# prstrive/SuRF

Hardware: AMD Instinct MI355X
Metric: rays/sec (576x800, 5-view, 128 samp/ray render, whole job) (higher is better)
Workload: dtype f32 (operands split exactly into 3 bf16 pieces, fp32 accumulate)

## Files before the change

include/surf_hip.h:

```cpp
#ifndef SURF_HIP_H
#define SURF_HIP_H

#include <stdint.h>

#ifdef __cplusplus
extern "C" {
#endif

#define SURF_MAX_VIEWS 8
#define SURF_MAX_STAGES 4
#define SURF_MAX_SAMPLES 256

#define SURF_E_ARG (-1)
#define SURF_E_LIMIT (-2)

#define SURF_ABI_VERSION 41
int surf_abi_version(void);

int surf_pack_texel4(const float* src, int n, int C, int H, int W, float* dst, void* stream);

int surf_ray_setup(const float* rays_o, const float* rays_d, const float* near, const float* far, int n_rays,
                   const float* mvol, int Dm, const float* lin_depth, int n_depth, const float* lin_samples,
                   const int* h_n_samples, const float* h_sample_ranges, int n_stage, const float* jitter,
                   float sample_dist, const int32_t* const* h_tables, const int* h_dims, int n_vol,
// ... 84 lines not shown
int surf_sdf_smooth_backward(const float* pts, const float* sbar, int64_t n, const float* const* h_vols,
                             const int32_t* const* h_tables, const int* h_dims, int n_vol, float* const* h_dvols,
                             const float* packed, float* in, float* ab, void* stream);

int surf_blend_raw_floats(void);
int surf_blend_packed_floats(void);
int surf_blend_pack_weights(const float* h_raw, float* h_packed);
int surf_blend(const float* pts, const uint8_t* mask, const int32_t* idx, int64_t n, const float* const* h_feats, const int* h_hw,
               int n_level, const float* imgs, int nv, const float* h_intrs, const float* h_w2c,
               const float* h_c2w, const float* blend_w, float* color, uint8_t* n_valid, void* stream);

#define SURF_BLEND_BF16X3 1
#define SURF_BLEND_F16X2 2
#define SURF_BLEND_F32 3
int64_t surf_blend_split_packed_bytes(int precision);
int surf_blend_pack_weights_split(const float* h_raw, unsigned char* h_packed, int precision);
int64_t surf_blend_split_scratch_bytes(int64_t n_points, int nv);
int surf_blend_split(const float* pts, const uint8_t* mask, const int32_t* idx, int64_t n, const float* const* h_feats,
                     const int* h_hw, int n_level, const float* imgs, int nv, const float* h_intrs, const float* h_w2c,
                     const float* h_c2w, const void* blend_w, int precision, float* color, uint8_t* n_valid, void* scratch,
                     void* stream);
int surf_blend_split_dn(const float* pts, const int32_t* idx, int64_t n_capacity, const int32_t* d_n, const float* const* h_feats,
                        const int* h_hw, int n_level, const float* imgs, int nv, const float* h_intrs, const float* h_w2c,
                        const float* h_c2w, const void* blend_w, int precision, float* color, uint8_t* n_valid, void* scratch,
                        void* stream);

int surf_composite(const float* sdf, const float* grad, const float* color, const uint8_t* n_valid,
                   const float* mid_z, const float* dists, const float* pts, const uint8_t* vmask,
                   const float* rays_d, int n_rays, int S, float inv_s, float cos_anneal_ratio,
                   const float* h_rot_ref, float* out_color, float* out_depth, float* out_sdf_depth,
                   float* out_normal, float* out_normal_val, uint8_t* out_valid, uint8_t* out_mid_inside,
                   float* out_weights, float* out_inside, float* out_eik, float* out_z_sdf0, void* stream);
int surf_composite_backward(const float* sdf, const float* grad, const float* color, const float* mid_z, const float* dists,
                            const float* pts, const uint8_t* vmask, const float* rays_d, int n_rays, int S, float inv_s,
                            float cos_anneal_ratio, const float* h_rot_ref, const float* g_color, const float* g_depth,
                            float eik_scale, float* d_sdf, float* d_grad, float* d_color, float* d_inv_s, void* stream);
int surf_composite_backward_s(const float* sdf, const float* grad, const float* color, const float* mid_z, const float* dists,
                              const float* pts, const uint8_t* vmask, const float* rays_d, int n_rays, int S, float inv_s,
                              float cos_anneal_ratio, const float* h_rot_ref, const float* g_color, const float* g_depth,
                              float eik_scale, const float* eik_upstream, float* d_sdf, float* d_grad, float* d_color,
                              float* d_inv_s, void* stream);



int surf_upsample_filter(const int32_t* parents, int64_t n_parents, int D, const float* depths, int nv, int H, int W,
                         const float* h_intrs, const float* h_w2c, float depth_range, uint8_t* flags, void* stream);

int surf_costvol(const int32_t* parents, const int32_t* idx, int64_t n, int D, const float* const* h_feats,
                 const int* h_hw, int stage, int nv, const float* h_intrs, const float* h_w2c, const float* h_agg,
                 int32_t* coords, float* feat, uint8_t* keep, void* stream);

int64_t surf_compact_workspace_ints(int64_t n);
int surf_compact(const uint8_t* flags, int64_t n, int32_t* workspace, int32_t* idx_out, int32_t* total, void* stream);

int surf_gather_rows(const void* src, const int32_t* idx, int64_t n, int row_words, int idx_shift, int dst_stride_words,
                     int dst_offset_words, void* dst, void* stream);
int surf_compose_index(const int32_t* a, const int32_t* b, int64_t n, int32_t* out, void* stream);

int surf_densify(const int32_t* coords, const float* rows, int row_stride, int64_t n, int D, const float* prev,
                 float* dense, int32_t* table, void* stream);

int surf_matching_depth(const float* mvol, int D, int nv, const float* h_kinv, const float* h_c2w, const float* h_rinv,
                        const float* h_near_fars, int H, int W, int h, int w, const float* lin_x, const float* lin_y,
                        const float* lin_n, int n, const float* pre_depths, float ratio_cur, float ratio_prev,
                        const float* jitter, float* depth_lr, float* depth_full, float* stats, void* stream);


int surf_spconv(const float* in, int cin, const int32_t* in_table, int D_in, const int32_t* out_coords, int64_t n_out,
                int mode, const float* weight, int cout, const float* bn_scale, const float* bn_shift, const float* skip,
                float* out, void* stream);
int surf_spconv_rows16(const uint16_t* in16, int cin, const int32_t* in_table, int D_in, const int32_t* out_coords, int64_t n_out,
                       int mode, const float* weight, int cout, float* out, void* stream);
int surf_rows_to_bf16(const float* x, int64_t n_floats, uint16_t* out16, void* stream);
int surf_bn_relu_apply16(const float* x, int64_t n, int channels, const float* scale, const float* shift, const float* skip,
                         float* out, uint16_t* out16, void* stream);
int surf_bn_relu_backward16(const float* x, const float* dy, int64_t n, int channels, const float* scale, const float* shift,
                            const float* mean, const float* invstd, int train, void* workspace, float* dgamma, float* dbeta,
                            float* dx, uint16_t* dx16, void* stream);
int64_t surf_spconv_packed_bytes(int cin, int cout);
int surf_spconv_pack_weights(const float* weight, int cin, int cout, void* packed, void* stream);
int surf_spconv_mfma(const float* in, int cin, const int32_t* in_table, int D_in, const int32_t* out_coords, int64_t n_out,
                     int mode, const void* packed, int cout, const float* bn_scale, const float* bn_shift,
                     const float* skip, float* out, int bf16_operands, void* stream);

int64_t surf_bn_workspace_bytes(int channels);
int surf_bn_train_affine(const float* x, int64_t n, int channels, const float* gamma, const float* beta, float eps,
                         float momentum, float* running_mean, float* running_var, float* scale, float* shift, float* batch_stats,
                         void* workspace, void* stream);
int surf_bn_relu_apply(const float* x, int64_t n, int channels, const float* scale, const float* shift, const float* skip,
                       float* out, void* stream);
int surf_bn_relu_backward(const float* x, const float* dy, int64_t n, int channels, const float* scale, const float* shift,
                          const float* mean, const float* invstd, int train, void* workspace, float* dgamma, float* dbeta,
                          float* dx, void* stream);
int64_t surf_inorm_backward_workspace_bytes(int N, int channels);
int surf_inorm_relu_backward(const float* x, const float* dy, int N, int64_t hw, int channels, const float* stats, void* workspace,
                             float* dx, void* stream);

int surf_matching_depth_backward(const float* mvol, int D, int nv, const float* h_kinv, const float* h_c2w, const float* h_rinv,
                                 const float* h_near_fars, int H, int W, int h, int w, const float* lin_x, const float* lin_y,
                                 const float* lin_n, int n, const float* pre_depths, float ratio_cur, float ratio_prev,
                                 const float* jitter, const float* g_full, int view0, int view1, float* g_lr, float* dmvol,
                                 const float* stats, void* stream);
int surf_densify_backward(const int32_t* coords, int64_t n, int D, const int32_t* table, const float* g_dense, int row_stride,
                          float* g_rows, float* g_prev, void* stream);
int surf_scatter_rows_add(const float* g_dst, const int32_t* idx, int64_t n, int row_words, int idx_shift, int dst_stride_words,
                          int dst_offset_words, float* g_src, void* stream);
// ... 162 lines not shown
```

surf_amd/csrc/volume.hip:

```cpp
#include <stdlib.h>

#include "common.h"

namespace {

struct ViewSet {
  int nv;
  float w2c[SURF_MAX_VIEWS][12];
  float K[SURF_MAX_VIEWS][12];
};

__constant__ int kChildOff[8][3] = {{0, 0, 0}, {1, 0, 0}, {0, 1, 0}, {0, 0, 1}, {1, 1, 0}, {1, 0, 1}, {0, 1, 1}, {1, 1, 1}};

__device__ __forceinline__ bool project_voxel(const ViewSet& vs, int v, float wx, float wy, float wz, float half_w,
                                              float half_h, float& nx, float& ny, float& qz) {
  const float* M = vs.w2c[v];
  float X = M[0] * wx + M[1] * wy + M[2] * wz + M[3];
  float Y = M[4] * wx + M[5] * wy + M[6] * wz + M[7];
  float Z = M[8] * wx + M[9] * wy + M[10] * wz + M[11];
  const float* K = vs.K[v];
  float qx = K[0] * X + K[1] * Y + K[2] * Z + K[3];
  float qy = K[4] * X + K[5] * Y + K[6] * Z + K[7];
  qz = K[8] * X + K[9] * Y + K[10] * Z + K[11];
  float x = qx / qz, y = qy / qz;
// ... 178 lines not shown
  __syncthreads();
  if (threadIdx.x == 0) block_counts[blockIdx.x] = s_part[0] + s_part[1] + s_part[2] + s_part[3];
}

__global__ __launch_bounds__(1024) void compact_scan_kernel(int32_t* __restrict__ block_counts, int nb,
                                                            int32_t* __restrict__ total) {
  __shared__ int s_buf[1024];
  __shared__ int s_carry;
  if (threadIdx.x == 0) s_carry = 0;
  __syncthreads();
  for (int c0 = 0; c0 < nb; c0 += 1024) {
    const int i = c0 + threadIdx.x;
    const int v = i < nb ? block_counts[i] : 0;
    s_buf[threadIdx.x] = v;
    __syncthreads();
    for (int o = 1; o < 1024; o <<= 1) {
      int t = threadIdx.x >= o ? s_buf[threadIdx.x - o] : 0;
      __syncthreads();
      s_buf[threadIdx.x] += t;
      __syncthreads();
    }
    const int incl = s_buf[threadIdx.x];
    const int carry = s_carry;
    if (i < nb) block_counts[i] = carry + incl - v;
    __syncthreads();
    if (threadIdx.x == 1023) s_carry = carry + incl;
    __syncthreads();
  }
  if (threadIdx.x == 0) *total = s_carry;
}

__global__ __launch_bounds__(CP_THREADS) void compact_scatter_kernel(const uint8_t* __restrict__ flags, int64_t n,
                                                                     const int32_t* __restrict__ block_offsets,
                                                                     int32_t* __restrict__ idx_out, bool aligned) {
  __shared__ int s_part[CP_THREADS / 64];
  const int lane = threadIdx.x & 63, wave = threadIdx.x >> 6;
  const int64_t base = (int64_t)blockIdx.x * CP_BLOCK + (int64_t)threadIdx.x * CP_ITEMS;
  const unsigned bits = cp_mask16(flags, base, n, aligned);
  const int c = __popc(bits);
  int incl = c;
#pragma unroll
  for (int o = 1; o < 64; o <<= 1) {
    int t = __shfl_up(incl, o);
    if (lane >= o) incl += t;
  }
  if (lane == 63) s_part[wave] = incl;
  __syncthreads();
  int wave_off = 0;
  for (int w = 0; w < wave; ++w) wave_off += s_part[w];
  int pos = block_offsets[blockIdx.x] + wave_off + incl - c;
#pragma unroll
  for (int k = 0; k < CP_ITEMS; ++k)
    if (bits & (1u << k)) idx_out[pos++] = (int32_t)(base + k);
}

__global__ __launch_bounds__(256) void gather_rows_kernel(const uint32_t* __restrict__ src, const int32_t* __restrict__ idx,
                                                          int64_t n, int w, int shift, int dst_stride, int dst_off,
                                                          uint32_t* __restrict__ dst) {
  const int64_t t = (int64_t)blockIdx.x * blockDim.x + threadIdx.x;
  if (t >= n * w) return;
  const int64_t i = t / w;
  const int c = (int)(t % w);
  dst[i * dst_stride + dst_off + c] = src[(int64_t)(idx[i] >> shift) * w + c];
}

__global__ __launch_bounds__(256) void compose_index_kernel(const int32_t* __restrict__ a, const int32_t* __restrict__ b,
                                                            int64_t n, int32_t* __restrict__ out) {
  const int64_t i = (int64_t)blockIdx.x * blockDim.x + threadIdx.x;
  if (i < n) out[i] = a[b[i]];
}

__device__ __forceinline__ void up2_src(int i, int Dp, int& i0, int& i1, float& l1) {
  float src = ((float)i + 0.5f) * 0.5f - 0.5f;
  if (src < 0.f) src = 0.f;
  i0 = (int)floorf(src);
  i1 = min(i0 + 1, Dp - 1);
  l1 = src - (float)i0;
}

template <int VEC, int NV>
__global__ __launch_bounds__(256) void dense_init_kernel(const float* __restrict__ prev, int D, float* __restrict__ dense,
                                                         int32_t* __restrict__ table) {
  const int64_t total = (int64_t)D * D * D;
  const int64_t t0 = (int64_t)blockIdx.x * (256 * NV) + threadIdx.x;
  const unsigned zc = (unsigned)D / VEC;
#pragma unroll
  for (int k = 0; k < NV; ++k) {
    const int64_t t = t0 + 256 * k, i0 = t * VEC;
    if (i0 >= total) return;
    const unsigned tu = (unsigned)t;
    const int zb = (int)(tu % zc) * VEC, y = (int)((tu / zc) % (unsigned)D), x = (int)(tu / (zc * (unsigned)D));
    float out[VEC];
    if (VEC == 4 && prev) {
      const int Dp = D / 2;
      int x0, x1, y0, y1;
      float lx, ly;
      up2_src(x, Dp, x0, x1, lx);
      up2_src(y, Dp, y0, y1, ly);
      const float hx = 1.0f - lx, hy = 1.0f - ly;
      const int c0 = zb / 2 - 1;
      float P[4][4];
#pragma unroll
      for (int t = 0; t < 4; ++t) {
        const int zc = min(max(c0 + t, 0), Dp - 1);
        P[0][t] = prev[((int64_t)x0 * Dp + y0) * Dp + zc];
        P[1][t] = prev[((int64_t)x0 * Dp + y1) * Dp + zc];
// ... 561 lines not shown
extern "C" int surf_upsample_filter(const int32_t* parents, int64_t n_parents, int D, const float* depths, int nv, int H,
                                    int W, const float* h_intrs, const float* h_w2c, float depth_range, uint8_t* flags,
                                    void* stream) {
  if (!parents || !depths || !h_intrs || !h_w2c || !flags || n_parents <= 0 || D < 2 || H < 2 || W < 2) return SURF_E_ARG;
  if (nv < 1 || nv > SURF_MAX_VIEWS) return SURF_E_LIMIT;
  FilterArgs a;
  a.parents = parents; a.n_par = n_parents; a.D = D; a.voxel_size = (float)(2.0 / (double)(D - 1));
  a.depths = depths; a.H = H; a.W = W; a.depth_range = depth_range; a.flags = flags;
  fill_views(a.vs, nv, h_intrs, h_w2c);
  hipLaunchKernelGGL(upsample_filter_kernel, grid1d(n_parents * 8, 256), dim3(256), 0, (hipStream_t)stream, a);
  return surf_check_launch();
}

extern "C" int surf_costvol(const int32_t* parents, const int32_t* idx, int64_t n, int D, const float* const* h_feats,
                            const int* h_hw, int stage, int nv, const float* h_intrs, const float* h_w2c,
                            const float* h_agg , int32_t* coords, float* feat,
                            uint8_t* keep, void* stream) {
  if (!h_feats || !h_hw || !h_intrs || !h_w2c || !h_agg || !coords || !feat || !keep || n <= 0 || D < 2) return SURF_E_ARG;
  if ((idx != nullptr) != (parents != nullptr)) return SURF_E_ARG;
  if (!idx && n != (int64_t)D * D * D) return SURF_E_ARG;
  if (nv < 1 || nv > SURF_MAX_VIEWS || stage < 0 || stage > 3) return SURF_E_LIMIT;
  CostVolArgs a;
  a.parents = parents; a.idx = idx; a.n = n; a.D = D; a.voxel_size = (float)(2.0 / (double)(D - 1)); a.stage = stage;
  for (int l = 0; l < 4; ++l) {
    if (!h_feats[l]) return SURF_E_ARG;
    a.feats[l] = h_feats[l];
    a.hw[2 * l] = h_hw[2 * l];
    a.hw[2 * l + 1] = h_hw[2 * l + 1];
  }
  fill_views(a.vs, nv, h_intrs, h_w2c);
  for (int k = 0; k < 32; ++k) a.w1[k] = h_agg[k];
  for (int k = 0; k < 8; ++k) { a.b1[k] = h_agg[32 + k]; a.w2[k] = h_agg[40 + k]; }
  a.b2 = h_agg[48];
  a.coords = coords; a.feat = feat; a.keep = keep;
  hipLaunchKernelGGL(costvol_kernel, grid1d(n, 256), dim3(256), 0, (hipStream_t)stream, a);
  return surf_check_launch();
}

extern "C" int64_t surf_compact_workspace_ints(int64_t n) { return (n + CP_BLOCK - 1) / CP_BLOCK + 1; }

extern "C" int surf_compact(const uint8_t* flags, int64_t n, int32_t* workspace, int32_t* idx_out, int32_t* total,
                            void* stream) {
  if (!flags || !workspace || !idx_out || !total || n <= 0) return SURF_E_ARG;
  if (n > 0x7fffffffLL) return SURF_E_LIMIT;
  const int nb = (int)((n + CP_BLOCK - 1) / CP_BLOCK);
  hipStream_t st = (hipStream_t)stream;
  const bool aligned = ((uintptr_t)flags & 15u) == 0;
  hipLaunchKernelGGL(compact_count_kernel, dim3(nb), dim3(CP_THREADS), 0, st, flags, n, workspace, aligned);
  hipLaunchKernelGGL(compact_scan_kernel, dim3(1), dim3(1024), 0, st, workspace, nb, total);
  hipLaunchKernelGGL(compact_scatter_kernel, dim3(nb), dim3(CP_THREADS), 0, st, flags, n, workspace, idx_out, aligned);
  return surf_check_launch();
}

extern "C" int surf_gather_rows(const void* src, const int32_t* idx, int64_t n, int row_words, int idx_shift,
                                int dst_stride_words, int dst_offset_words, void* dst, void* stream) {
  if (!src || !idx || !dst || n <= 0 || row_words <= 0 || idx_shift < 0 || dst_stride_words < row_words) return SURF_E_ARG;
  hipLaunchKernelGGL(gather_rows_kernel, grid1d(n * row_words, 256), dim3(256), 0, (hipStream_t)stream,
                     (const uint32_t*)src, idx, n, row_words, idx_shift, dst_stride_words, dst_offset_words, (uint32_t*)dst);
  return surf_check_launch();
}

extern "C" int surf_compose_index(const int32_t* a, const int32_t* b, int64_t n, int32_t* out, void* stream) {
  if (!a || !b || !out || n <= 0) return SURF_E_ARG;
  hipLaunchKernelGGL(compose_index_kernel, grid1d(n, 256), dim3(256), 0, (hipStream_t)stream, a, b, n, out);
  return surf_check_launch();
}

extern "C" int surf_densify(const int32_t* coords, const float* rows, int row_stride, int64_t n, int D, const float* prev,
                            float* dense, int32_t* table, void* stream) {
  if (!coords || !rows || !dense || !table || n <= 0 || D < 2 || row_stride < 1) return SURF_E_ARG;
  if (prev && (D & 1)) return SURF_E_ARG;
  hipStream_t st = (hipStream_t)stream;
  if (D % 4 == 0)
    hipLaunchKernelGGL((dense_init_kernel<4, 4>), grid1d((int64_t)D * D * D / 4, 256 * 4), dim3(256), 0, st, prev, D, dense, table);
  else
    hipLaunchKernelGGL((dense_init_kernel<1, 4>), grid1d((int64_t)D * D * D, 256 * 4), dim3(256), 0, st, prev, D, dense, table);
  hipLaunchKernelGGL(dense_scatter_kernel, grid1d(n, 256), dim3(256), 0, st, coords, rows, row_stride, n, D, dense, table);
  return surf_check_launch();
}

extern "C" int surf_densify_backward(const int32_t* coords, int64_t n, int D, const int32_t* table, const float* g_dense,
                                     int row_stride, float* g_rows, float* g_prev, void* stream) {
  if (!coords || !table || !g_dense || !g_rows || n <= 0 || D < 2 || row_stride < 1) return SURF_E_ARG;
  if (g_prev && (D & 1)) return SURF_E_ARG;
  hipStream_t st = (hipStream_t)stream;
  hipLaunchKernelGGL(dense_rows_bwd_kernel, grid1d(n, 256), dim3(256), 0, st, coords, g_dense, n, D, row_stride, g_rows);
  if (g_prev)
  {
    const int64_t total = (int64_t)D * D * D;
    const int Dp = D / 2;
    const int64_t tiles = (int64_t)((Dp + DG_TX - 1) / DG_TX) * ((Dp + DG_TY - 1) / DG_TY) * ((Dp + DG_TZ - 1) / DG_TZ);
#ifndef SURF_DENSE_BWD_SCATTER
    if (tiles <= 0x7fffffffLL && Dp >= 2)
      hipLaunchKernelGGL(dense_init_bwd_gather_kernel, dim3((unsigned)tiles), dim3(256), 0, st, g_dense, table, D, g_prev);
    else
#endif
    if (D % 4 == 0)
      hipLaunchKernelGGL((dense_init_bwd_kernel<4, 8>), grid1d(total / 4, 256 * 8), dim3(256), 0, st, g_dense, table, D, g_prev);
    else
      hipLaunchKernelGGL((dense_init_bwd_kernel<1, 8>), grid1d(total, 256 * 8), dim3(256), 0, st, g_dense, table, D, g_prev);
  }
  return surf_check_launch();
}

extern "C" int surf_scatter_rows_add(const float* g_dst, const int32_t* idx, int64_t n, int row_words, int idx_shift,
                                     int dst_stride_words, int dst_offset_words, float* g_src, void* stream) {
// ... 88 lines not shown
```

surf_amd/implicit_surface.py:

```python
import math

import numpy as np
import torch
import torch.nn as nn

from . import ops
from .grads import accumulate


class _WNLinear(nn.Module):

    def __init__(self, weight, bias):
        super().__init__()
        self.weight_g = nn.Parameter(torch.linalg.norm(weight, dim=1, keepdim=True).clone())
        self.weight_v = nn.Parameter(weight.clone())
        self.bias = nn.Parameter(bias.clone())


class SDFNetworkSparse(nn.Module):

    def __init__(self, d_in=3, d_out=129, d_hidden=128, n_layers=6, skip_in=(3,), multires=4, bias=0.5, scale=1.0,
                 geometric_init=True, weight_norm=True, inside_outside=False, feat_channels=28, feat_multires=0):
        super().__init__()
        if not (d_in == 3 and d_hidden == 128 and n_layers == 6 and tuple(skip_in) == (3,) and multires == 4
                and feat_channels == 28 and feat_multires == 0 and float(scale) == 1.0 and weight_norm):
            raise NotImplementedError("the HIP SDF kernel implements the architecture shipped in confs/*.conf "
                                      "(d_hidden 128, n_layers 6, skip_in [3], multires 4, feat_channels 28, scale 1)")
        self.scale = scale
        in0 = 3 + 3 * 2 * multires
        dims = [in0] + [d_hidden + feat_channels] * n_layers + [d_out]
        self.num_layers = len(dims)
        for l in range(self.num_layers - 1):
            out_dim = dims[l + 1] - dims[0] if (l + 1) in skip_in else dims[l + 1]
            if l < self.num_layers - 2:
                out_dim -= feat_channels
            lin = nn.Linear(dims[l], out_dim)
            if geometric_init:
                with torch.no_grad():
                    if l == self.num_layers - 2:
                        sgn = -1.0 if inside_outside else 1.0
                        nn.init.normal_(lin.weight, mean=sgn * math.sqrt(math.pi) / math.sqrt(dims[l]), std=0.0001)
                        nn.init.constant_(lin.bias, -sgn * bias)
                        lin.weight[:, -feat_channels:] = 0.0
                        lin.bias[-feat_channels:] = 0.0
                    elif l == 0:
                        nn.init.constant_(lin.bias, 0.0)
                        lin.weight[:, 3:] = 0.0
                        nn.init.normal_(lin.weight[:, :3], 0.0, math.sqrt(2) / math.sqrt(out_dim))
                    elif l in skip_in:
                        nn.init.constant_(lin.bias, 0.0)
                        nn.init.normal_(lin.weight, 0.0, math.sqrt(2) / math.sqrt(out_dim))
                        lin.weight[:, -(dims[0] - 3 + feat_channels):] = 0.0
                    else:
# ... 47 lines not shown
        self.mvol = mv.contiguous().float()
        self.sv = ops.SparseVolumes([v.detach().float() for v in volumes], list(sparse_idxes))
        self.feats_t4 = [ops.pack_texel4(f.detach().float().contiguous()) for f in features]
        self.imgs_t4 = ops.pack_texel4(imgs.detach().float().contiguous())
        self.cams = ops.Cameras(intrs, c2ws)
        self.device = dev
        self.match_feats_t4 = None
        self._warp_maps = {}

    def occupied_any(self, pts):
        return ops.occupied_any(pts.float().contiguous(), self.sv)

    def warp_maps(self, use_match=False):
        key = bool(use_match and self.match_feats_t4 is not None)
        if key and getattr(self, "match_ready", None) is not None:
            ops.side.wait_for(self.match_ready)
            self.match_ready = None
        if key not in self._warp_maps:
            f = self.match_feats_t4 if key else self.feats_t4
            H, W = f[0].shape[1:3]
            self._warp_maps[key] = [f[0], ops.upsample_bilinear_t4(f[1], H, W), ops.upsample_bilinear_t4(f[2], H, W)]
        return self._warp_maps[key]

    @classmethod
    def from_device_layouts(cls, mvol, volumes, tables, feats_t4, imgs_t4, cams):
        self = cls.__new__(cls)
        self.mvol = mvol
        self.sv = ops.SparseVolumes(list(volumes), list(tables))
        self.feats_t4 = list(feats_t4)
        self.imgs_t4 = imgs_t4
        self.cams = cams
        self.device = mvol.device
        self.match_feats_t4 = None
        self._warp_maps = {}
        return self


class _LatticeScene:

    def __init__(self, volumes, sparse_idxes):
        self.sv = ops.SparseVolumes([v.detach().float() for v in volumes], list(sparse_idxes))
        self.device = self.sv.vols[0].device


def _occupied_list(rec, key):
    lst = rec.get(key + "_idx")
    if lst is None:
        lst = rec[key + "_idx"] = rec[key].nonzero().squeeze(1)
    return lst


MESH_EXTRACTIONS = ("dense", "band")
MESH_BAND_MARGIN = 2.0


class ImplicitSurface(nn.Module):

    def __init__(self, confs):
        super().__init__()
        self.n_samples = [int(n) for n in confs.get_list("render.n_samples")]
        self.sample_ranges = [float(r) for r in confs.get_list("render.sample_ranges")]
        self.n_depth = confs.get_int("render.n_depth")
        self.perturb = confs.get_float("render.perturb")
        self.val_chunk = confs.get_int("render.val_chunk", 1 << 19)
        self.sdf_network = SDFNetworkSparse(**dict(confs["sdf_network"]))
        self.color_network = BlendingNetwork(**dict(confs["color_network"]))
        self.deviation_network = SingleVarianceNetwork(**dict(confs["variance_network"]))
        self.sdf_precision = confs.get_string("render.sdf_precision", "bf16x3")
        if self.sdf_precision not in ops.SDF_PRECISIONS:
            raise ValueError(f"render.sdf_precision must be one of {ops.SDF_PRECISIONS}, got {self.sdf_precision!r}")
        self.blend_precision = confs.get_string("render.blend_precision", ops.BLEND_DEFAULT)
        if self.blend_precision not in ops.BLEND_PRECISIONS:
            raise ValueError(f"render.blend_precision must be one of {ops.BLEND_PRECISIONS}, got {self.blend_precision!r}")
        self.mesh_extraction = confs.get_string("render.mesh_extraction", "dense")
        if self.mesh_extraction not in MESH_EXTRACTIONS:
            raise ValueError(f"render.mesh_extraction must be one of {MESH_EXTRACTIONS}, got {self.mesh_extraction!r}")
        self.mesh_band_margin = confs.get_float("render.mesh_band_margin", MESH_BAND_MARGIN)
        if not self.mesh_band_margin >= 0.0:
            raise ValueError(f"render.mesh_band_margin must be >= 0, got {self.mesh_band_margin!r}")
        self.mesh_vertex_attributes = bool(confs.get_bool("render.vertex_attributes", False))
        self._packed = None
        self.kernel_events = None
        self.active_samples_log = None
        self.last_active_samples = None
        self.register_load_state_dict_post_hook(lambda module, incompatible: module.invalidate_packed())

    def invalidate_packed(self):
        self._packed = None
        if getattr(self.sdf_network, "_surf_flat", None) is not None:
            object.__setattr__(self.sdf_network, "_surf_flat", None)

    def train(self, mode=True):
        self.invalidate_packed()
        return super().train(mode)

    def packed_weights(self, device):
        ver = tuple((p._version, p.data_ptr()) for p in self.parameters()) + (str(device), self.sdf_precision, self.blend_precision)
        if self._packed is None or self._packed[0] != ver:
            from . import packing
            on_device = next(self.parameters()).is_cuda and packing.supported(self.sdf_precision, self.blend_precision)
            if on_device:
                with torch.no_grad():
                    sdf_w = packing.sdf_pack_split_device(self.sdf_network, self.sdf_precision)
                    blend_w = packing.blend_pack_split_device(self.color_network, self.blend_precision)
            else:
                sd = {k: v for k, v in self.state_dict().items()}
                sdf_w = (ops.sdf_pack_weights(sd, device, "sdf_network.") if self.sdf_precision == "f32" else
                         ops.sdf_pack_weights_split(sd, device, "sdf_network.", self.sdf_precision))
                blend_w = ops.blend_pack_weights(sd, device, "color_network.", self.blend_precision)
            self._packed = (ver, sdf_w, blend_w)
        return self._packed[1], self._packed[2]

    def smooth_weights(self, device):
        self.packed_weights(device)
        if len(self._packed) == 3:
            if next(self.parameters()).is_cuda:
                from . import packing
                with torch.no_grad():
                    sm = packing.sdf_pack_smooth_device(self.sdf_network)
            else:
                sm = ops.sdf_smooth_pack_weights({k: v for k, v in self.state_dict().items()}, device, "sdf_network.")
            self._packed = self._packed + (sm,)
        return self._packed[3]

    def scene(self, matching_volume, volumes, sparse_idxes, mask_volumes, features, imgs, intrs, c2ws):
        return SceneVolumes(matching_volume, volumes, sparse_idxes, features, imgs, intrs, c2ws)

    def render_scene(self, rays_o, rays_d, near, far, scene, cos_anneal_ratio=1.0, per_sample=True, jitter=None,
                     patch_warp=False, step=None):
        dev = rays_o.device
        self._random_pts = None
        if jitter is None and self.perturb > 0:
            jitter = self.draw_jitter(rays_o.shape[0])
        if jitter is not None:
            jitter = jitter.to(dev, torch.float32).contiguous()
        sdf_w, blend_w = self.packed_weights(dev)
        rays_o = rays_o.float().contiguous()
        rays_d = rays_d.float().contiguous()
        ev = self.kernel_events

        def timed(name, fn):
            if ev is None:
                return fn()
            a, b = torch.cuda.Event(enable_timing=True), torch.cuda.Event(enable_timing=True)
            a.record()
            r = fn()
            b.record()
            ev.append((name, a, b))
            return r

        st = timed("ray_setup", lambda: ops.ray_setup(rays_o, rays_d, near.float(), far.float(), scene.mvol, scene.sv,
                                                      self.n_samples, self.sample_ranges, self.n_depth, jitter=jitter,
                                                      want_z=patch_warp))
        n_act = None
        if patch_warp or self.sdf_precision == "f32" or self.blend_precision == "f32":
            act = timed("compact", lambda: ops.compact(st["vmask"]))
            if patch_warp and act.shape[0] == 0:
                act = torch.arange(min(10, st["vmask"].numel()), dtype=torch.int32, device=dev)
        else:
            act, n_act = timed("compact", lambda: ops.compact_counted(st["vmask"]))
        side_fwd = None
        if patch_warp:
            def smooth_branch():
                smooth, _ = ops.sdf_smooth(st["pts"], scene.sv, self.smooth_weights(dev), active_idx=act)
                inside = ((torch.linalg.norm(st["pts"], ord=2, dim=-1) < 1.0) & st["vmask"].bool()).float()
                err = (torch.linalg.norm(smooth, ord=2, dim=-1) * inside).sum() / (inside.sum() + 1e-5)
                return smooth, inside, err

            def sparse_branch():
                pr = self._random_pts if self._random_pts is not None else torch.rand([1024, 3]) * 2 - 1
                pr = pr.to(dev, torch.float32).contiguous()
                occ = scene.occupied_any(pr)
                sdf_r, _ = ops.sdf_mlp(pr, scene.sv, sdf_w, mask=occ.to(torch.uint8), want_grad=False)
                return pr, occ, torch.where(occ, sdf_r, torch.zeros_like(sdf_r))

            if ops.side.active("fwd") and dev.type == "cuda" and ev is None:
                self.smooth_weights(dev)
                side_fwd = (ops.side.run(smooth_branch, lane=1), ops.side.run(sparse_branch, lane=0))
        sdf, grad = timed("sdf_mlp", lambda: ops.sdf_mlp(st["pts"], scene.sv, sdf_w, mask=st["vmask"], active_idx=act,
                                                         active_count=n_act))
        col, nvalid = timed("blend", lambda: ops.blend(st["pts"], scene.feats_t4, scene.imgs_t4, scene.cams, blend_w,
                                                       mask=st["vmask"], active_idx=act, active_count=n_act))
        out = timed("composite", lambda: ops.composite(sdf, grad, col, nvalid, st, rays_d, self.deviation_network.inv_s(),
                                                       float(cos_anneal_ratio), scene.cams, per_sample=per_sample,
                                                       want_z0=patch_warp))
        if ev is not None:
            self.last_active_samples = int(act.shape[0]) if n_act is None else n_act
            if self.active_samples_log is not None:
                self.active_samples_log.append(self.last_active_samples)
        R, S = st["mid_z"].shape
        eik = out.pop("eik").sum(dim=0)
        out["gradient_error"] = eik[0] / (eik[1] + 1e-5)
        out["valid_mask"] = out["valid_mask"].bool()
        out["mid_inside_sphere"] = out["mid_inside_sphere"].float()
        out["mid_z_vals"] = st["mid_z"]
        if per_sample:
            out["gradients"] = grad.view(R, S, 3)
            out["sdf"] = sdf.view(R, S)
        out["s_val"] = torch.full((1, 1), 1.0 / self.deviation_network.inv_s(), device=dev)
        if patch_warp:
            pts0 = ops.surface_points(rays_o, rays_d, out.pop("z_sdf0"), st["z_vals"])
            _, g0 = ops.sdf_mlp(pts0, scene.sv, sdf_w)
            maps = scene.warp_maps(use_match=not (step is None or step < 2))
            out["ref_gray_val"], out["sampled_gray_val"] = ops.patch_warp(pts0, g0, maps, scene.cams)
            out["pts_sdf0"], out["gradients_sdf0"] = pts0, g0
            ops.side.join(lanes=(0, 1, 3))
            if side_fwd is not None:
                (smooth, inside, out["smooth_error"]), (pr, occ, sdf_r0) = side_fwd
            else:
                smooth, inside, out["smooth_error"] = smooth_branch()
                pr, occ, sdf_r0 = sparse_branch()
            out["sparse_sdf"] = torch.cat([sdf_r0, sdf]).view(-1, 1)
            self._ctx = dict(st=st, act=act, sdf=sdf, grad=grad, col=col, rays_d=rays_d, anneal=float(cos_anneal_ratio),
# ... 373 lines not shown
```

surf_amd/ops.py:

```python
import ctypes
import os

import numpy as np
import torch

from . import _lib

BLEND_KEYS = ["s"] + [f"{m}.{i}.{p}" for m, idxs in (("ray_dir_fc", (0, 2)), ("base_fc", (0, 2)), ("vis_fc", (0, 2)),
                                                      ("vis_fc2", (0, 2)), ("rgb_fc", (0, 2, 4)))
                      for i in idxs for p in ("weight", "bias")]


def _stream():
    return ctypes.c_void_p(torch.cuda.current_stream().cuda_stream)


kernel_events = None


class _timed:

    def __init__(self, name, units=0):
        self.name, self.units = name, units

# ... 892 lines not shown




def _cams_ext(cams, intrs, c2ws):
    if not hasattr(cams, "kinv"):
        i_cpu = intrs.detach().to("cpu", torch.float32)
        c_cpu = c2ws.detach().to("cpu", torch.float32)
        cams.kinv = np.ascontiguousarray(torch.inverse(i_cpu)[:, :3, :3].contiguous().numpy())
        cams.rinv = np.ascontiguousarray(torch.inverse(c_cpu[:, :3, :3]).contiguous().numpy())
    return cams


def upsample_filter(parents, D, depths, cams, depth_range):
    _chk(parents, torch.int32, "parents")
    _chk(depths, torch.float32, "depths")
    nv, H, W = depths.shape
    flags = torch.empty(parents.shape[0] * 8, dtype=torch.uint8, device=parents.device)
    _lib.lib().surf_upsample_filter(_p(parents), parents.shape[0], int(D), _p(depths), nv, H, W, _np_ptr(cams.intrs),
                                    _np_ptr(cams.w2c), float(depth_range), _p(flags), _stream())
    return flags


def agg_mlp_host(sd, prefix="volume."):
    return np.concatenate([_host_f32(sd[prefix + k]).reshape(-1) for k in
                           ("agg_mlp.0.weight", "agg_mlp.0.bias", "agg_mlp.2.weight", "agg_mlp.2.bias")])


def costvol(feats_t4_c2f, stage, D, cams, agg, parents=None, idx=None):
    dev = feats_t4_c2f[0].device
    n = int(D) ** 3 if idx is None else int(idx.shape[0])
    coords = torch.empty(n, 3, dtype=torch.int32, device=dev)
    feat = torch.empty(n, 8, dtype=torch.float32, device=dev)
    keep = torch.empty(n, dtype=torch.uint8, device=dev)
    hw = (ctypes.c_int * 8)(*[int(v) for f in feats_t4_c2f for v in f.shape[1:3]])
    fp = _ptr_array(feats_t4_c2f)
    agg = np.ascontiguousarray(agg, dtype=np.float32)
    _lib.lib().surf_costvol(_p(parents), _p(idx), n, int(D), fp, hw, int(stage), cams.nv, _np_ptr(cams.intrs),
                            _np_ptr(cams.w2c), _np_ptr(agg), _p(coords), _p(feat), _p(keep), _stream())
    return coords, feat, keep


def compact(flags):
    _chk(flags, torch.uint8, "flags")
    n = flags.numel()
    dev = flags.device
    ws = torch.empty(_lib.lib().surf_compact_workspace_ints(n), dtype=torch.int32, device=dev)
    idx = torch.empty(n, dtype=torch.int32, device=dev)
    total = torch.empty(1, dtype=torch.int32, device=dev)
    _lib.lib().surf_compact(_p(flags), n, _p(ws), _p(idx), _p(total), _stream())
    return idx[:int(total.item())]


def compact_counted(flags):
    _chk(flags, torch.uint8, "flags")
    n = flags.numel()
    dev = flags.device
    ws = torch.empty(_lib.lib().surf_compact_workspace_ints(n), dtype=torch.int32, device=dev)
    idx = torch.empty(n, dtype=torch.int32, device=dev)
    total = torch.empty(1, dtype=torch.int32, device=dev)
    _lib.lib().surf_compact(_p(flags), n, _p(ws), _p(idx), _p(total), _stream())
    return idx, total


def gather_rows(src, idx, shift=0, dst=None, dst_off=0):
    assert src.is_contiguous() and src.element_size() == 4 and src.is_cuda
    _chk(idx, torch.int32, "idx")
    w = src.shape[1]
    n = idx.shape[0]
    if dst is None:
        dst = torch.empty(n, w, dtype=src.dtype, device=src.device)
    _lib.lib().surf_gather_rows(_p(src), _p(idx), n, w, int(shift), dst.shape[1], int(dst_off), _p(dst), _stream())
    return dst


def compose_index(a, b):
    out = torch.empty_like(b)
    _lib.lib().surf_compose_index(_p(a), _p(b), b.shape[0], _p(out), _stream())
    return out


def densify(coords, rows, D, prev=None):
    _chk(coords, torch.int32, "coords")
    _chk(rows, torch.float32, "rows")
    dev = coords.device
    dense = torch.empty(D, D, D, dtype=torch.float32, device=dev)
    table = torch.empty(D, D, D, dtype=torch.int32, device=dev)
    _lib.lib().surf_densify(_p(coords), _p(rows), rows.shape[1], coords.shape[0], int(D), _p(prev), _p(dense), _p(table), _stream())
    return dense, table


def matching_depth(mvol, cams, near_fars, H, W, res_level, n, pre_depths=None, ratio_cur=1.0, ratio_prev=1.0, return_lr=False,
                   jitter=None, saved=None):
    _chk(mvol, torch.float32, "matching volume")
    dev = mvol.device
    h, w = H // res_level, W // res_level
    lin_x = _linspace_dev(0, W - 1, w, dev)
    lin_y = _linspace_dev(0, H - 1, h, dev)
    lin_n = _linspace_dev(0.0, 1.0, n, dev)
    nf = _near_fars_host(near_fars)
    lr = torch.empty(cams.nv, h, w, dtype=torch.float32, device=dev)
    full = torch.empty(cams.nv, H, W, dtype=torch.float32, device=dev)
    if jitter is not None:
        _chk(jitter, torch.float32, "jitter")
        assert tuple(jitter.shape) == (cams.nv, h * w, 2)
    stats = torch.empty(cams.nv, h, w, 4, dtype=torch.float32, device=dev) if saved is not None else None
    _lib.lib().surf_matching_depth(_p(mvol), int(mvol.shape[0]), cams.nv, _np_ptr(cams.kinv), _np_ptr(cams.c2w),
                                   _np_ptr(cams.rinv), _np_ptr(nf), H, W, h, w, _p(lin_x), _p(lin_y), _p(lin_n), int(n),
                                   _p(pre_depths), float(ratio_cur), float(ratio_prev),
                                   _p(jitter), _p(lr), _p(full), _p(stats), _stream())
    if saved is not None:
        saved["stats"] = stats
    return (full, lr) if return_lr else full

# ... 1085 lines not shown
```

Measured before the change: 3.292 million.

## Compact active samples in ray-group/sample-block order for locality

Adds a blocked stream-compaction variant that emits active sample indices grouped as blocks of G rays by B consecutive samples instead of plain ray-major order. The default config (8 rays x 4 samples) routes the render's compaction through it, so downstream per-sample kernels (MLP, smoothing, gathers) process spatially neighbouring samples from nearby rays together, aiming for better cache and feature-volume locality. The cost is extra index arithmetic in the compaction kernels and a different ordering that downstream consumers must tolerate.

```diff
diff --git a/include/surf_hip.h b/include/surf_hip.h
--- a/include/surf_hip.h
+++ b/include/surf_hip.h
@@ -160,6 +160,8 @@
 
 int64_t surf_compact_workspace_ints(int64_t n);
 int surf_compact(const uint8_t* flags, int64_t n, int32_t* workspace, int32_t* idx_out, int32_t* total, void* stream);
+int surf_compact_blocked(const uint8_t* flags, int64_t n_rays, int64_t n_samples, int rays_per_block, int samples_per_block,
+                         int32_t* workspace, int32_t* idx_out, int32_t* total, void* stream);
 
 int surf_gather_rows(const void* src, const int32_t* idx, int64_t n, int row_words, int idx_shift, int dst_stride_words,
                      int dst_offset_words, void* dst, void* stream);
diff --git a/surf_amd/csrc/volume.hip b/surf_amd/csrc/volume.hip
--- a/surf_amd/csrc/volume.hip
+++ b/surf_amd/csrc/volume.hip
@@ -254,6 +254,130 @@
 #pragma unroll
   for (int k = 0; k < CP_ITEMS; ++k)
     if (bits & (1u << k)) idx_out[pos++] = (int32_t)(base + k);
+}
+
+struct CpBlocked {
+  int R, S, G, B, log_b;
+};
+
+struct CpWalk {
+  int blk, gb, sb, g, j;
+  __device__ __forceinline__ void seek(uint32_t p, const CpBlocked& a) {
+    const uint32_t per_blk = (uint32_t)a.G * (uint32_t)a.S;
+    blk = (int)(p / per_blk);
+    const uint32_t q = p - (uint32_t)blk * per_blk;
+    gb = min(a.G, a.R - blk * a.G);
+    const uint32_t chunk = (uint32_t)gb << a.log_b;
+    sb = (int)(q / chunk);
+    const uint32_t r = q - (uint32_t)sb * chunk;
+    g = (int)(r >> a.log_b);
+    j = (int)(r & (uint32_t)(a.B - 1));
+  }
+  __device__ __forceinline__ int32_t flat(const CpBlocked& a) const { return (blk * a.G + g) * a.S + (sb << a.log_b) + j; }
+  template <int W>
+  __device__ __forceinline__ void step(const CpBlocked& a) {
+    j += W;
+    if (j < a.B) return;
+    j = 0;
+    if (++g < gb) return;
+    g = 0;
+    if ((++sb << a.log_b) < a.S) return;
+    sb = 0;
+    ++blk;
+    gb = min(a.G, a.R - blk * a.G);
+  }
+};
+
+template <int W>
+__device__ __forceinline__ unsigned cp_mask_w(const uint8_t* __restrict__ p, bool aligned) {
+  unsigned bits = 0;
+  if (W >= 4 && aligned) {
+    uint32_t w[W >= 4 ? W / 4 : 1];
+    if constexpr (W == 16) {
+      const uint4 v = *reinterpret_cast<const uint4*>(p);
+      w[0] = v.x; w[1] = v.y; w[2] = v.z; w[3] = v.w;
+    } else if constexpr (W == 8) {
+      const uint2 v = *reinterpret_cast<const uint2*>(p);
+      w[0] = v.x; w[1] = v.y;
+    } else {
+      w[0] = *reinterpret_cast<const uint32_t*>(p);
+    }
+#pragma unroll
+    for (int k = 0; k < W; ++k) bits |= (((w[k >> 2] >> (8 * (k & 3))) & 0xffu) ? 1u : 0u) << k;
+  } else {
+#pragma unroll
+    for (int k = 0; k < W; ++k) bits |= (p[k] ? 1u : 0u) << k;
+  }
+  return bits;
+}
+
+template <int W>
+__device__ __forceinline__ unsigned cp_blocked_mask16(const uint8_t* __restrict__ flags, int64_t base, int64_t n,
+                                                      const CpBlocked& a, bool aligned, int32_t (&first)[CP_ITEMS / W]) {
+  unsigned bits = 0;
+#pragma unroll
+  for (int k = 0; k < CP_ITEMS / W; ++k) first[k] = 0;
+  if (base >= n) return 0;
+  CpWalk w;
+  w.seek((uint32_t)base, a);
+#pragma unroll
+  for (int k = 0; k < CP_ITEMS / W; ++k) {
+    if (base + k * W < n) {
+      first[k] = w.flat(a);
+      bits |= cp_mask_w<W>(flags + first[k], aligned) << (k * W);
+      w.template step<W>(a);
+    }
+  }
+  return bits;
+}
+
+template <int W>
+__global__ __launch_bounds__(CP_THREADS) void compact_blocked_count_kernel(const uint8_t* __restrict__ flags, int64_t n, CpBlocked a,
+                                                                           int32_t* __restrict__ block_counts, bool aligned) {
+  __shared__ int s_part[CP_THREADS / 64];
+  const int64_t base = (int64_t)blockIdx.x * CP_BLOCK + (int64_t)threadIdx.x * CP_ITEMS;
+  int32_t first[CP_ITEMS / W];
+  int c = __popc(cp_blocked_mask16<W>(flags, base, n, a, aligned, first));
+  c = (int)wave_sum((float)c);
+  if ((threadIdx.x & 63) == 0) s_part[threadIdx.x >> 6] = c;
+  __syncthreads();
+  if (threadIdx.x == 0) block_counts[blockIdx.x] = s_part[0] + s_part[1] + s_part[2] + s_part[3];
+}
+
+template <int W>
+__global__ __launch_bounds__(CP_THREADS) void compact_blocked_scatter_kernel(const uint8_t* __restrict__ flags, int64_t n, CpBlocked a,
+                                                                             const int32_t* __restrict__ block_offsets,
+                                                                             int32_t* __restrict__ idx_out, bool aligned) {
+  __shared__ int s_part[CP_THREADS / 64];
+  const int lane = threadIdx.x & 63, wave = threadIdx.x >> 6;
+  const int64_t base = (int64_t)blockIdx.x * CP_BLOCK + (int64_t)threadIdx.x * CP_ITEMS;
+  int32_t first[CP_ITEMS / W];
+  const unsigned bits = cp_blocked_mask16<W>(flags, base, n, a, aligned, first);
+  const int c = __popc(bits);
+  int incl = c;
+#pragma unroll
+  for (int o = 1; o < 64; o <<= 1) {
+    int t = __shfl_up(incl, o);
+    if (lane >= o) incl += t;
+  }
+  if (lane == 63) s_part[wave] = incl;
+  __syncthreads();
+  int wave_off = 0;
+  for (int w = 0; w < wave; ++w) wave_off += s_part[w];
+  int pos = block_offsets[blockIdx.x] + wave_off + incl - c;
+#pragma unroll
+  for (int k = 0; k < CP_ITEMS; ++k)
+    if (bits & (1u << k)) idx_out[pos++] = first[k / W] + (k % W);
+}
+
+template <int W>
+static void compact_blocked_launch(const uint8_t* flags, int64_t n, const CpBlocked& a, int32_t* workspace, int32_t* idx_out,
+                                   int32_t* total, hipStream_t st) {
+  const int nb = (int)((n + CP_BLOCK - 1) / CP_BLOCK);
+  const bool aligned = ((uintptr_t)flags & 15u) == 0;
+  hipLaunchKernelGGL(compact_blocked_count_kernel<W>, dim3(nb), dim3(CP_THREADS), 0, st, flags, n, a, workspace, aligned);
+  hipLaunchKernelGGL(compact_scan_kernel, dim3(1), dim3(1024), 0, st, workspace, nb, total);
+  hipLaunchKernelGGL(compact_blocked_scatter_kernel<W>, dim3(nb), dim3(CP_THREADS), 0, st, flags, n, a, workspace, idx_out, aligned);
 }
 
 __global__ __launch_bounds__(256) void gather_rows_kernel(const uint32_t* __restrict__ src, const int32_t* __restrict__ idx,
@@ -921,6 +1045,26 @@
   return surf_check_launch();
 }
 
+extern "C" int surf_compact_blocked(const uint8_t* flags, int64_t n_rays, int64_t n_samples, int rays_per_block,
+                                    int samples_per_block, int32_t* workspace, int32_t* idx_out, int32_t* total, void* stream) {
+  const int64_t G = rays_per_block, B = samples_per_block;
+  if (!flags || !workspace || !idx_out || !total || n_rays <= 0 || n_samples <= 0) return SURF_E_ARG;
+  if (G <= 0 || B <= 0 || (G & (G - 1)) || (B & (B - 1)) || n_samples % B) return SURF_E_ARG;
+  const int64_t n = n_rays * n_samples;
+  if (n_rays > 0x7fffffffLL || n_samples > 0x7fffffffLL || n + G * n_samples > 0x7fffffffLL) return SURF_E_LIMIT;
+  CpBlocked a;
+  a.R = (int)n_rays; a.S = (int)n_samples; a.G = (int)G; a.B = (int)B;
+  a.log_b = 0;
+  while ((1 << a.log_b) < a.B) ++a.log_b;
+  hipStream_t st = (hipStream_t)stream;
+  if (B >= 16) compact_blocked_launch<16>(flags, n, a, workspace, idx_out, total, st);
+  else if (B == 8) compact_blocked_launch<8>(flags, n, a, workspace, idx_out, total, st);
+  else if (B == 4) compact_blocked_launch<4>(flags, n, a, workspace, idx_out, total, st);
+  else if (B == 2) compact_blocked_launch<2>(flags, n, a, workspace, idx_out, total, st);
+  else compact_blocked_launch<1>(flags, n, a, workspace, idx_out, total, st);
+  return surf_check_launch();
+}
+
 extern "C" int surf_gather_rows(const void* src, const int32_t* idx, int64_t n, int row_words, int idx_shift,
                                 int dst_stride_words, int dst_offset_words, void* dst, void* stream) {
   if (!src || !idx || !dst || n <= 0 || row_words <= 0 || idx_shift < 0 || dst_stride_words < row_words) return SURF_E_ARG;
diff --git a/surf_amd/implicit_surface.py b/surf_amd/implicit_surface.py
--- a/surf_amd/implicit_surface.py
+++ b/surf_amd/implicit_surface.py
@@ -1,4 +1,5 @@
 import math
+import os
 
 import numpy as np
 import torch
@@ -152,6 +153,7 @@
 
 MESH_EXTRACTIONS = ("dense", "band")
 MESH_BAND_MARGIN = 2.0
+SAMPLE_BLOCK = (8, 4)
 
 
 class ImplicitSurface(nn.Module):
@@ -179,6 +181,13 @@
         if not self.mesh_band_margin >= 0.0:
             raise ValueError(f"render.mesh_band_margin must be >= 0, got {self.mesh_band_margin!r}")
         self.mesh_vertex_attributes = bool(confs.get_bool("render.vertex_attributes", False))
+        blk = confs.get_list("render.sample_block", list(SAMPLE_BLOCK))
+        if os.environ.get("SURF_SAMPLE_BLOCK"):
+            blk = os.environ["SURF_SAMPLE_BLOCK"].split(",")
+        self.sample_block = tuple(int(v) for v in blk)
+        G, B = self.sample_block if len(self.sample_block) == 2 else (0, 0)
+        if G < 1 or G & (G - 1) or B < 0 or B & (B - 1) or (B == 0 and G != 1):
+            raise ValueError(f"render.sample_block must be [G, B] with powers of two ([1, 0]: ray-major), got {list(blk)!r}")
         self._packed = None
         self.kernel_events = None
         self.active_samples_log = None
@@ -258,7 +267,10 @@
             if patch_warp and act.shape[0] == 0:
                 act = torch.arange(min(10, st["vmask"].numel()), dtype=torch.int32, device=dev)
         else:
-            act, n_act = timed("compact", lambda: ops.compact_counted(st["vmask"]))
+            S = st["mid_z"].shape[1]
+            G, B = self.sample_block
+            blk = (S, G, B) if B > 0 and S % B == 0 else None
+            act, n_act = timed("compact", lambda: ops.compact_counted(st["vmask"], block=blk))
         side_fwd = None
         if patch_warp:
             def smooth_branch():
diff --git a/surf_amd/ops.py b/surf_amd/ops.py
--- a/surf_amd/ops.py
+++ b/surf_amd/ops.py
@@ -968,14 +968,20 @@
     return idx[:int(total.item())]
 
 
-def compact_counted(flags):
+def compact_counted(flags, block=None):
     _chk(flags, torch.uint8, "flags")
     n = flags.numel()
     dev = flags.device
     ws = torch.empty(_lib.lib().surf_compact_workspace_ints(n), dtype=torch.int32, device=dev)
     idx = torch.empty(n, dtype=torch.int32, device=dev)
     total = torch.empty(1, dtype=torch.int32, device=dev)
-    _lib.lib().surf_compact(_p(flags), n, _p(ws), _p(idx), _p(total), _stream())
+    if block is None:
+        _lib.lib().surf_compact(_p(flags), n, _p(ws), _p(idx), _p(total), _stream())
+    else:
+        S, G, B = (int(v) for v in block)
+        if S <= 0 or n % S:
+            raise ValueError(f"compact_counted: {n} flags are no whole number of rays of {S} samples")
+        _lib.lib().surf_compact_blocked(_p(flags), n // S, S, G, B, _p(ws), _p(idx), _p(total), _stream())
     return idx, total
 
 
```

Measured after the change: 3.356 million (median of 6 runs). +2.0%, better.
